# ModelTC/Dipoorlet

Measured on AMD Instinct MI355X. Metric: calibration images/sec (whole node) + achieved HBM GB/s, ResNet-50 ONNX N=1024, -A hist, higher is better.
Workload: dtype f32; 1 GPU; ResNet-50 ONNX activation set (T=123, 26598376 fp32 elems/img), -A hist --bins 2048, N=1024 per GPU in 32 batches of 32: range pass + histogram pass + percentile clip; device=AMD Radeon Graphics (gfx950:sramecc+:xnack-), hist_checksum_ok=True, world_size_seen_by_backend=1

## Files before the change

### dipoorlet_amd/_hip.py

```python
import ctypes as C
import os

import torch

_HERE = os.path.dirname(os.path.abspath(__file__))
LIB_PATH = os.environ.get("DPL_LIB") or os.path.join(_HERE, "csrc", "libdipoorlet_hip.so")

ABI_VERSION = 24
MAX_BINS = 16384
HIST_SPEC_MAX_TENSORS = 2048


class Span(C.Structure):
    _fields_ = [("offset", C.c_uint64), ("count", C.c_uint64), ("seg", C.c_uint32), ("slot", C.c_uint32)]


class WorkItem(C.Structure):
    _fields_ = [("offset", C.c_uint64), ("count", C.c_uint32), ("seg", C.c_uint32), ("slot", C.c_uint32),
                ("reserved", C.c_uint32)]


class HistRange(C.Structure):
    _fields_ = [("first", C.c_float), ("last", C.c_float), ("step", C.c_float), ("inv", C.c_float),
                ("zero_bin", C.c_uint32), ("status", C.c_uint32), ("dmax", C.c_float), ("exact_div", C.c_uint32)]
# ... 44 lines not shown
SIGNATURES = {
    "dpl_abi_version": (C.c_int, []),
    "dpl_last_error": (C.c_char_p, []),
    "dpl_device_info": (C.c_int, [C.c_char_p, C.c_int, C.POINTER(C.c_int), C.POINTER(C.c_uint64)]),
    "dpl_stream_priority_range": (C.c_int, [C.POINTER(C.c_int), C.POINTER(C.c_int)]),
    "dpl_stream_create": (C.c_int, [C.c_int, C.POINTER(C.c_void_p)]),
    "dpl_stream_destroy": (C.c_int, [_P]),
    "dpl_build_work_items": (_I64, [_P, _I64, _U64, _P, _I64]),
    "dpl_build_balanced_items": (_I64, [_P, _I64, _I64, _P, _I64, _P]),
    "dpl_minmax_init": (C.c_int, [_P, _P, _P, _I64, _P]),
    "dpl_minmax_accumulate": (C.c_int, [_P, _I64, _P, _I64, _P, _P, _P, _P, _P]),
    "dpl_minmax_finalize": (C.c_int, [_P, _P, _P, _I64, _P, _P, _P]),
    "dpl_minmax_encode": (C.c_int, [_P, _P, _I64, _P, _P, _P, _P]),
    "dpl_hist_prepare": (C.c_int, [_P, _P, _I64, C.c_int, _P, _P]),
    "dpl_abs_hist_accumulate": (C.c_int, [_P, _I64, _P, _I64, _P, _P, C.c_int, _P, _P]),
    "dpl_hist_spec_entry_bytes": (_U64, [_I64, C.c_int]),
    "dpl_minmax_hist_accumulate": (C.c_int, [_P, _I64, _P, _I64, _P, _P, _P, _P, _I64, C.c_int, _P, _P]),
    "dpl_hist_spec_accumulate": (C.c_int, [_P, _P, _I64, _I64, _P, _P, C.c_int, _P, _P, _P]),
    "dpl_hist_spec_cuts": (C.c_int, [_P, _P, _I64, _I64, _P, _P]),
    "dpl_hist_percentile": (C.c_int, [_P, _P, _P, _I64, C.c_int, _DBL, _P, _P]),
    "dpl_hist_kl": (C.c_int, [_P, _P, _P, _I64, C.c_int, C.c_int, _P, _P, _P, _P]),
    "dpl_octav_init": (C.c_int, [_P, _I64, C.c_int, _P]),
    "dpl_octav_run_compact": (C.c_int, [_P, _I64, _P, _I64, _P, _P, _I64, _P, _P, _P, _P, _P, C.c_int, C.c_int, _P]),
    "dpl_octav_run": (C.c_int, [_P, _I64, _P, _I64, _P, _P, _I64, C.c_int, C.c_int, _P]),
    "dpl_octav_run_bracket": (C.c_int, [_P, _I64, _P, _I64, _P, _P, _I64, _P, _P, _P, _P, _P, _P, _P, _P, C.c_int,
                                        C.c_int, _P]),
    "dpl_octav_slice_cap": (C.c_uint32, []),
    "dpl_octav_small_pair": (C.c_uint32, []),
    "dpl_build_octav_slices": (_I64, [_P, _I64, _P, _I64, _P]),
    "dpl_octav_oneread_prepare": (C.c_int, [_P, _P]),
    "dpl_octav_oneread_stream": (C.c_int, [_P, _P]),
    "dpl_octav_oneread_finish": (C.c_int, [_P, _P]),
    "dpl_octav_oneread_compaction": (C.c_int, [_P, _P]),
# ... 120 lines not shown
```

### dipoorlet_amd/csrc/calib_kernels.hip

```cpp
#include "common.hpp"

#pragma clang fp contract(off)

namespace {

struct MinMaxOp {
    float mn, mx;
    uint32_t nan;
    __device__ __forceinline__ void operator()(float x) {
        mn = fminf(mn, x);
        mx = fmaxf(mx, x);
        nan |= (x != x);
    }
};

__device__ __forceinline__ void minmax_commit(const MinMaxOp& op, uint32_t slot, float* s_mn, float* s_mx, uint32_t* s_nan,
                                              uint32_t* __restrict__ min_enc, uint32_t* __restrict__ max_enc,
                                              uint32_t* __restrict__ nan_flag) {
    float mn = wave_min(op.mn), mx = wave_max(op.mx);
    uint32_t nn = __any(op.nan) ? 1u : 0u;
    const int w = threadIdx.x / kWave;
    if ((threadIdx.x & (kWave - 1)) == 0) {
        s_mn[w] = mn;
        s_mx[w] = mx;
// ... 105 lines not shown
};

template <bool kFast>
__device__ __forceinline__ void hist_op_init(HistOp<kFast>& op, const dpl_hist_range& r, int bins, uint32_t* lds) {
    op.lds = lds;
    op.first = r.first;
    op.last = r.last;
    op.step = r.step;
    op.inv = r.inv;
    op.denom = __fsub_rn(r.last, r.first);
    op.last_bin = bins - 1;
    op.fbins = (float)bins;
    op.nonzero = 0u;
}

template <class Count>
__device__ __forceinline__ void hist_flush(uint32_t nonzero, const dpl_work_item& it, const dpl_hist_range& r, int bins,
                                           Count* __restrict__ hist, uint32_t* lds, uint32_t* s_nz) {
    const uint32_t nzw = wave_sum(nonzero);
    if ((threadIdx.x & (kWave - 1)) == 0) s_nz[threadIdx.x / kWave] = nzw;
    __syncthreads();
    if (threadIdx.x == 0) {
        uint32_t nzb = 0;
        for (int k = 0; k < kBlock / kWave; ++k) nzb += s_nz[k];
        const uint32_t z = it.count - nzb;
        if (z) atomicAdd(lds + r.zero_bin, z);
        const uint32_t top = lds[bins];
        if (top) atomicAdd(lds + bins - 1, top);
    }
    __syncthreads();
    Count* __restrict__ out = hist + (uint64_t)it.slot * (uint64_t)bins;
    for (int b = threadIdx.x; b < bins; b += kBlock) {
        const uint32_t c = lds[b];
        if (c) {
            if constexpr (sizeof(Count) == 8)
                atomicAdd(reinterpret_cast<unsigned long long*>(out + b), (unsigned long long)c);
            else
                atomicAdd(out + b, c);
        }
    }
}

template <bool kFast>
__device__ __forceinline__ void hist_body(const dpl_work_item& it, const float* const* __restrict__ segs,
                                          const dpl_hist_range& r, int bins, uint64_t* __restrict__ hist,
                                          uint32_t* lds, uint32_t* s_nz) {
    HistOp<kFast> op;
    hist_op_init(op, r, bins, lds);
    stream_span(segs[it.seg] + it.offset, it.count, op);
    hist_flush(op.nonzero, it, r, bins, hist, lds, s_nz);
}

__global__ __launch_bounds__(kBlock) void k_abs_hist(const dpl_work_item* __restrict__ items,
                                                      const uint32_t* __restrict__ bb,
                                                      const float* const* __restrict__ segs,
// ... 52 lines not shown
        b = b < 0 ? 0 : b;
        if (a < hist_edge(b, r.step, first)) --b;
        if (b != bins - 1 && a >= hist_edge(b + 1, r.step, first)) ++b;
        r.zero_bin = (uint32_t)(b < 0 ? 0 : b);
    }
    return r;
}

__global__ void k_hist_prepare(const float* __restrict__ gmin, const float* __restrict__ gmax, int64_t n, int bins,
                               dpl_hist_range* __restrict__ out) {
    int64_t i = (int64_t)blockIdx.x * blockDim.x + threadIdx.x;
    if (i >= n) return;
    out[i] = hist_range_of(gmin[i], gmax[i], bins);
}

__host__ __device__ inline uint64_t spec_counts_offset(int64_t n_slots) {
    return (((uint64_t)n_slots * (sizeof(dpl_hist_range) + sizeof(uint32_t))) + 15ull) & ~15ull;
}

__global__ __launch_bounds__(kBlock) void k_hist_snapshot(const uint32_t* __restrict__ mn, const uint32_t* __restrict__ mx,
                                                           const uint32_t* __restrict__ nan, int64_t n, int bins,
                                                           dpl_hist_range* __restrict__ snap, uint32_t* __restrict__ flags,
                                                           uint32_t* __restrict__ counts) {
    const int64_t i = (int64_t)blockIdx.x * blockDim.x + threadIdx.x;
    const int64_t stride = (int64_t)gridDim.x * blockDim.x;
    if (i < n) {
        float gmin, gmax;
        minmax_decode(mn[i], mx[i], nan[i], gmin, gmax);
        snap[i] = hist_range_of(gmin, gmax, bins);
        flags[i] = 0u;
    }
    const int64_t total = n * (int64_t)bins;
    for (int64_t j = i; j < total; j += stride) counts[j] = 0u;
}

template <bool kFast>
struct MinMaxHistOp {
    MinMaxOp m;
    HistOp<kFast> h;
    __device__ __forceinline__ void operator()(float x) {
        m(x);
        h(x);
    }
};

template <bool kFast>
__device__ __forceinline__ void minmax_hist_body(const dpl_work_item& it, const float* const* __restrict__ segs,
                                                 const dpl_hist_range& r, int bins, uint32_t* __restrict__ counts,
                                                 uint32_t* lds, uint32_t* s_nz, MinMaxOp& m) {
    MinMaxHistOp<kFast> op;
    op.m = m;
    hist_op_init(op.h, r, bins, lds);
    stream_span(segs[it.seg] + it.offset, it.count, op);
    m = op.m;
    hist_flush(op.h.nonzero, it, r, bins, counts, lds, s_nz);
}

__global__ __launch_bounds__(kBlock) void k_minmax_hist(const dpl_work_item* __restrict__ items,
                                                         const uint32_t* __restrict__ bb,
                                                         const float* const* __restrict__ segs,
                                                         uint32_t* __restrict__ min_enc, uint32_t* __restrict__ max_enc,
                                                         uint32_t* __restrict__ nan_flag,
                                                         const dpl_hist_range* __restrict__ snap, int bins,
                                                         uint32_t* __restrict__ counts) {
    extern __shared__ __attribute__((aligned(16))) uint32_t lds_mh[];
    uint32_t* s_nz = lds_mh + bins + 1;
    float* s_mn = reinterpret_cast<float*>(s_nz + kBlock / kWave);
    float* s_mx = s_mn + kBlock / kWave;
    uint32_t* s_nan = reinterpret_cast<uint32_t*>(s_mx + kBlock / kWave);
    uint32_t k0, k1;
    block_items(bb, k0, k1);
    for (uint32_t k = k0; k < k1; ++k) {
        const dpl_work_item it = items[k];
        const dpl_hist_range r = snap[it.slot];
        MinMaxOp m{INFINITY, -INFINITY, 0u};
        if (r.status != 0u) {
            stream_span(segs[it.seg] + it.offset, it.count, m);
        } else {
            for (int b = threadIdx.x; b <= bins; b += kBlock) lds_mh[b] = 0u;
            __syncthreads();
            if (r.exact_div)
                minmax_hist_body<false>(it, segs, r, bins, counts, lds_mh, s_nz, m);
            else
                minmax_hist_body<true>(it, segs, r, bins, counts, lds_mh, s_nz, m);
        }
        minmax_commit(m, it.slot, s_mn, s_mx, s_nan, min_enc, max_enc, nan_flag);
    }
}

__global__ __launch_bounds__(kBlock) void k_hist_resolve(const dpl_hist_range* __restrict__ snap,
                                                          const dpl_hist_range* __restrict__ fin,
                                                          const uint32_t* __restrict__ counts, const uint64_t* __restrict__ elems,
                                                          int bins, uint64_t* __restrict__ hist, uint32_t* __restrict__ flags,
                                                          unsigned long long* __restrict__ stats) {
    const uint32_t t = blockIdx.x;
    const uint32_t* a = reinterpret_cast<const uint32_t*>(snap + t);
    const uint32_t* b = reinterpret_cast<const uint32_t*>(fin + t);
    bool same = true;
#pragma unroll
    for (int w = 0; w < (int)(sizeof(dpl_hist_range) / 4); ++w) same = same && (a[w] == b[w]);
    const uint32_t status = fin[t].status;
    const bool valid = same && status == 0u;
    if (threadIdx.x == 0) {
        flags[t] = valid ? 1u : (status != 0u ? 2u : 0u);
        if (stats) {
            const unsigned long long e = elems[t];
            atomicAdd(stats + 0, 1ull);
            atomicAdd(stats + 2, e);
            if (valid) {
                atomicAdd(stats + 1, 1ull);
                atomicAdd(stats + 3, e);
            }
        }
    }
    if (!valid) return;
    const uint32_t* __restrict__ row = counts + (uint64_t)t * (uint64_t)bins;
    uint64_t* __restrict__ out = hist + (uint64_t)t * (uint64_t)bins;
    for (int j = threadIdx.x; j < bins; j += kBlock) {
        const uint32_t c = row[j];
        if (c) out[j] += (uint64_t)c;
    }
}

__device__ __forceinline__ uint64_t shfl_up_u64(uint64_t v, int d) {
    const uint32_t lo = __shfl_up((uint32_t)v, d, kWave), hi = __shfl_up((uint32_t)(v >> 32), d, kWave);
    return ((uint64_t)hi << 32) | lo;
}

__device__ __forceinline__ void rest_prefix(const uint64_t* __restrict__ elems, const uint32_t* __restrict__ flags, int n_tensors,
                                            uint64_t* P, uint64_t* s_tot) {
    const int per = (n_tensors + kBlock - 1) / kBlock;
    const int t0 = (int)threadIdx.x * per;
    uint64_t mine = 0;
    for (int j = 0; j < per; ++j) {
        const int t = t0 + j;
        if (t < n_tensors && flags[t] == 0u) mine += elems[t];
    }
    uint64_t incl = mine;
    const int lane = threadIdx.x & (kWave - 1), wv = threadIdx.x / kWave;
#pragma unroll
    for (int o = 1; o < kWave; o <<= 1) {
        const uint64_t up = shfl_up_u64(incl, o);
        if (lane >= o) incl += up;
    }
    if (lane == kWave - 1) s_tot[wv] = incl;
    __syncthreads();
    uint64_t run = incl - mine;
    for (int w = 0; w < wv; ++w) run += s_tot[w];
    for (int j = 0; j < per; ++j) {
        const int t = t0 + j;
        if (t < n_tensors) {
            P[t] = run;
            if (flags[t] == 0u) run += elems[t];
        }
    }
    if (threadIdx.x == kBlock - 1) P[n_tensors] = run;
    __syncthreads();
}

__device__ __forceinline__ void rest_cut(const uint64_t* P, int n_tensors, uint64_t G, uint64_t b, uint64_t& cut, int& at) {
    const uint64_t total = P[n_tensors], q = total / G, rem = total % G;
    const uint64_t target = (b >= G) ? total : q * b + (rem * b) / G;
    if (target >= total) {
        cut = total;
        at = n_tensors;
        return;
    }
    int lo = 1, hi = n_tensors;
    while (lo < hi) {
        const int mid = (lo + hi) >> 1;
        if (P[mid] > target) hi = mid; else lo = mid + 1;
    }
    at = lo - 1;
    cut = P[lo - 1] + ((target - P[lo - 1]) & ~1023ull);
}

__global__ __launch_bounds__(kBlock) void k_abs_hist_rest(const uint64_t* __restrict__ elems, const uint32_t* __restrict__ flags,
                                                           int n_tensors, const float* const* __restrict__ segs,
                                                           const dpl_hist_range* __restrict__ ranges, int bins,
                                                           uint64_t* __restrict__ hist) {
    extern __shared__ __attribute__((aligned(16))) uint32_t lds_rest[];
    uint64_t* P = reinterpret_cast<uint64_t*>(lds_rest);
    uint64_t* s_tot = P + n_tensors + 1;
    uint32_t* lds = reinterpret_cast<uint32_t*>(s_tot + kBlock / kWave);
    uint32_t* s_nz = lds + bins + 1;
    rest_prefix(elems, flags, n_tensors, P, s_tot);
    if (P[n_tensors] == 0) return;
    uint64_t cut[2];
    int at[2];
    rest_cut(P, n_tensors, gridDim.x, blockIdx.x, cut[0], at[0]);
    rest_cut(P, n_tensors, gridDim.x, (uint64_t)blockIdx.x + 1, cut[1], at[1]);
    uint64_t pos = cut[0];
    const uint64_t end = cut[1];
    int t = at[0];
    while (pos < end) {
        while (P[t + 1] <= pos) ++t;
        const uint64_t stop = P[t + 1] < end ? P[t + 1] : end;
        dpl_work_item it;
        it.offset = pos - P[t];
        it.count = (uint32_t)(stop - pos);
        it.seg = (uint32_t)t;
// ... 4 lines not shown
        __syncthreads();
        if (r.exact_div)
            hist_body<false>(it, segs, r, bins, hist, lds, s_nz);
        else
            hist_body<true>(it, segs, r, bins, hist, lds, s_nz);
        __syncthreads();
        pos = stop;
    }
}

__global__ __launch_bounds__(kBlock) void k_hist_spec_cuts(const uint64_t* __restrict__ elems, const uint32_t* __restrict__ flags,
                                                            int n_tensors, uint64_t* __restrict__ cuts) {
    extern __shared__ __attribute__((aligned(16))) uint32_t lds_cuts[];
    uint64_t* P = reinterpret_cast<uint64_t*>(lds_cuts);
    uint64_t* s_tot = P + n_tensors + 1;
    rest_prefix(elems, flags, n_tensors, P, s_tot);
    if (threadIdx.x != 0) return;
    uint64_t cut = 0;
    int at = 0;
    if (P[n_tensors] != 0) rest_cut(P, n_tensors, gridDim.x, blockIdx.x, cut, at);
    cuts[blockIdx.x] = cut;
    if (blockIdx.x + 1 == gridDim.x) cuts[gridDim.x] = P[n_tensors];
}

__device__ __forceinline__ void store_bin_clip(int found, float gmin, float gmax, int bins, float* __restrict__ clip) {
    float lo = gmin, hi = gmax;
    if (found >= 0) {
        const float dmax = py_max(-gmin, gmax);
        const float cv = __fmul_rn((float)found + 0.5f, __fdiv_rn(dmax, (float)bins));
        lo = py_max(-cv, gmin);
        hi = py_min(cv, gmax);
// ... 767 lines not shown
}

int dpl_abs_hist_accumulate(const dpl_work_item* d_items, int64_t n_items, const uint32_t* d_block_begin,
                            int64_t n_blocks, const float* const* d_seg_ptrs, const dpl_hist_range* d_ranges,
                            int bins, uint64_t* d_hist, dpl_stream_t s) {
    if (bins < 1 || bins > DPL_MAX_BINS) return fail_msg("dpl_abs_hist_accumulate: bins must be in [1, 16384]");
    if (n_items <= 0) return 0;
    if (int e = check_blocks("dpl_abs_hist_accumulate", n_items, d_block_begin, n_blocks)) return e;
    hipLaunchKernelGGL(k_abs_hist, dim3((unsigned)n_blocks), dim3(kBlock),
                       ((size_t)bins + 1 + kBlock / kWave) * sizeof(uint32_t), (hipStream_t)s, d_items, d_block_begin,
                       d_seg_ptrs, d_ranges, bins, d_hist);
    DPL_LAUNCH_CHECK("k_abs_hist");
    return 0;
}

uint64_t dpl_hist_spec_entry_bytes(int64_t n_slots, int bins) {
    if (n_slots < 0 || bins < 1 || bins > DPL_MAX_BINS) return 0;
    return spec_counts_offset(n_slots) + (uint64_t)n_slots * (uint64_t)bins * sizeof(uint32_t);
}

int dpl_minmax_hist_accumulate(const dpl_work_item* d_items, int64_t n_items, const uint32_t* d_block_begin,
                               int64_t n_blocks, const float* const* d_seg_ptrs, uint32_t* d_min_enc, uint32_t* d_max_enc,
                               uint32_t* d_nan, int64_t n_slots, int bins, void* d_entry, dpl_stream_t s) {
    if (bins < 1 || bins > DPL_MAX_BINS) return fail_msg("dpl_minmax_hist_accumulate: bins must be in [1, 16384]");
    if (!d_entry || ((uintptr_t)d_entry & 15u)) return fail_msg("dpl_minmax_hist_accumulate: d_entry must be 16-byte aligned");
    if (n_slots <= 0 || n_slots > 0x7FFFFFFFll) return fail_msg("dpl_minmax_hist_accumulate: n_slots out of range");
    if (n_items <= 0) return 0;
    if (int e = check_blocks("dpl_minmax_hist_accumulate", n_items, d_block_begin, n_blocks)) return e;
    dpl_hist_range* snap = (dpl_hist_range*)d_entry;
    uint32_t* flags = (uint32_t*)(snap + n_slots);
    uint32_t* counts = (uint32_t*)((char*)d_entry + spec_counts_offset(n_slots));
    int64_t zb = grid_for(n_slots * (int64_t)bins, kBlock * 8);
    if (zb < grid_for(n_slots, kBlock)) zb = grid_for(n_slots, kBlock);
    if (zb > 1024) zb = 1024;
    hipLaunchKernelGGL(k_hist_snapshot, dim3((unsigned)zb), dim3(kBlock), 0, (hipStream_t)s, d_min_enc, d_max_enc, d_nan,
                       n_slots, bins, snap, flags, counts);
    DPL_LAUNCH_CHECK("k_hist_snapshot");
    hipLaunchKernelGGL(k_minmax_hist, dim3((unsigned)n_blocks), dim3(kBlock),
                       ((size_t)bins + 1 + 4 * (kBlock / kWave)) * sizeof(uint32_t), (hipStream_t)s, d_items, d_block_begin,
                       d_seg_ptrs, d_min_enc, d_max_enc, d_nan, snap, bins, counts);
    DPL_LAUNCH_CHECK("k_minmax_hist");
    return 0;
}

int dpl_hist_spec_accumulate(void* d_entry, const uint64_t* d_elems, int64_t n_slots, int64_t n_blocks,
                             const float* const* d_seg_ptrs, const dpl_hist_range* d_ranges, int bins, uint64_t* d_hist,
                             uint64_t* d_stats, dpl_stream_t s) {
    if (bins < 1 || bins > DPL_MAX_BINS) return fail_msg("dpl_hist_spec_accumulate: bins must be in [1, 16384]");
    if (!d_entry || ((uintptr_t)d_entry & 15u)) return fail_msg("dpl_hist_spec_accumulate: d_entry must be 16-byte aligned");
    if (n_slots <= 0 || n_slots > DPL_HIST_SPEC_MAX_TENSORS)
        return fail_msg("dpl_hist_spec_accumulate: n_slots must be in [1, DPL_HIST_SPEC_MAX_TENSORS]");
    if (n_blocks <= 0 || n_blocks > 0x7FFFFFFFll) return fail_msg("dpl_hist_spec_accumulate: n_blocks out of range");
    dpl_hist_range* snap = (dpl_hist_range*)d_entry;
    uint32_t* flags = (uint32_t*)(snap + n_slots);
    const uint32_t* counts = (const uint32_t*)((char*)d_entry + spec_counts_offset(n_slots));
    hipLaunchKernelGGL(k_hist_resolve, dim3((unsigned)n_slots), dim3(kBlock), 0, (hipStream_t)s, snap, d_ranges, counts, d_elems,
                       bins, d_hist, flags, (unsigned long long*)d_stats);
    DPL_LAUNCH_CHECK("k_hist_resolve");
    const size_t lds = ((size_t)n_slots + 1 + kBlock / kWave) * sizeof(uint64_t) + ((size_t)bins + 1 + kBlock / kWave) * sizeof(uint32_t);
    hipLaunchKernelGGL(k_abs_hist_rest, dim3((unsigned)n_blocks), dim3(kBlock), lds, (hipStream_t)s, d_elems, flags, (int)n_slots,
                       d_seg_ptrs, d_ranges, bins, d_hist);
    DPL_LAUNCH_CHECK("k_abs_hist_rest");
    return 0;
}

int dpl_hist_spec_cuts(const void* d_entry, const uint64_t* d_elems, int64_t n_slots, int64_t n_blocks, uint64_t* d_cuts,
                       dpl_stream_t s) {
    if (!d_entry || !d_cuts) return fail_msg("dpl_hist_spec_cuts: null argument");
    if (n_slots <= 0 || n_slots > DPL_HIST_SPEC_MAX_TENSORS)
        return fail_msg("dpl_hist_spec_cuts: n_slots must be in [1, DPL_HIST_SPEC_MAX_TENSORS]");
    if (n_blocks <= 0 || n_blocks > 0x7FFFFFFFll) return fail_msg("dpl_hist_spec_cuts: n_blocks out of range");
    const uint32_t* flags = (const uint32_t*)((const dpl_hist_range*)d_entry + n_slots);
    hipLaunchKernelGGL(k_hist_spec_cuts, dim3((unsigned)n_blocks), dim3(kBlock),
                       ((size_t)n_slots + 1 + kBlock / kWave) * sizeof(uint64_t), (hipStream_t)s, d_elems, flags, (int)n_slots, d_cuts);
    DPL_LAUNCH_CHECK("k_hist_spec_cuts");
    return 0;
// ... 117 lines not shown
```

### dipoorlet_amd/ops.py

```python
import ctypes as C
import os
import weakref

import numpy as np
import torch

from . import _hip

_SEG_CACHE_MAX = 64


def _stream():
    return C.c_void_p(torch.cuda.current_stream().cuda_stream)


def _ptr(t):
    return C.c_void_p(t.data_ptr())


def _require_cuda(t, name="tensor"):
    if not (isinstance(t, torch.Tensor) and t.is_cuda):
        raise _hip.DipoorletHipError(f"{name} must be a ROCm device tensor; dipoorlet_amd has no CPU path")
    if t.dtype != torch.float32 or not t.is_contiguous():
        raise _hip.DipoorletHipError(f"{name} must be contiguous float32")


def _upload_struct_array(arr, n, device):
    nbytes = C.sizeof(arr._type_) * max(n, 1)
    host = torch.frombuffer(bytearray(C.string_at(C.addressof(arr), nbytes)), dtype=torch.uint8)
    return host.to(device)


DEFAULT_BLOCKS = {"minmax": 256, "hist": 768, "octav": 1024, "cos": 512, "fq": 65536}


class WorkSet:

    def __init__(self, items, n_items, block_begin, n_blocks):
        self.items, self.n_items, self.block_begin, self.n_blocks = items, n_items, block_begin, n_blocks

    def args(self):
        bb = _ptr(self.block_begin) if self.block_begin is not None else C.c_void_p(0)
        return _ptr(self.items), self.n_items, bb, self.n_blocks


class TensorSetPlan:

    def __init__(self, elems_per_image, batch, device, chunk_elems=None):
# ... 3 lines not shown
        self.device = torch.device(device)
        self.total = sum(self.elems) * self.batch
        self.chunk = int(chunk_elems) if chunk_elems else None
        self._work = {}
        self._seg_cache = {}

    @property
    def n_pairs(self):
        return self.batch * self.T

    def _spans(self, per_image):
        if per_image:
            return [(t, b * e, e, b * self.T + t) for b in range(self.batch) for t, e in enumerate(self.elems)]
        return [(t, 0, e * self.batch, t) for t, e in enumerate(self.elems)]

    def work(self, kind, per_image=False):
        nb = None if self.chunk else max(1, min(DEFAULT_BLOCKS[kind], (self.total + 4095) // 4096))
        key = (per_image, nb)
        w = self._work.get(key)
        if w is None:
            spans = self._spans(per_image)
            if self.chunk:
                arr, n = _hip.build_work_items(spans, self.chunk)
                w = WorkSet(_upload_struct_array(arr, n, self.device), n, None, n)
            else:
                arr, n, bb = _hip.build_balanced_items(spans, nb)
                bbt = torch.frombuffer(bytearray(bytes(bb)), dtype=torch.int32).to(self.device)
                w = WorkSet(_upload_struct_array(arr, n, self.device), n, bbt, nb)
            self._work[key] = w
        return w

    def elems_device(self):
# ... 195 lines not shown
            raise _hip.DipoorletHipError(f"bins must be in [1, {_hip.MAX_BINS}]")
        self.min_enc = torch.empty(self.n, dtype=torch.int32, device=self.device)
        self.max_enc = torch.empty(self.n, dtype=torch.int32, device=self.device)
        self.nan = torch.empty(self.n, dtype=torch.int32, device=self.device)
        self.gmin = torch.empty(self.n, dtype=torch.float32, device=self.device)
        self.gmax = torch.empty(self.n, dtype=torch.float32, device=self.device)
        self.hist = None
        self.ranges = None
        self.speculate = bool(speculate)
        self._ledger = {}
        self._slab = []
        self._spec_stats = torch.zeros(4, dtype=torch.int64, device=self.device) if self.speculate else None
        self.reset_minmax()

    def reset_minmax(self):
        for _, entry, _ in self._ledger.values():
            self._slab.append(entry)
        self._ledger.clear()
        _hip.check(_hip.lib().dpl_minmax_init(_ptr(self.min_enc), _ptr(self.max_enc), _ptr(self.nan), self.n,
                                              _stream()), "dpl_minmax_init")

    def will_speculate(self, plan, tensors, per_image=False):
        return (self.speculate and isinstance(tensors, BoundSet) and not per_image and plan.chunk is None
                and 0 < plan.T <= min(self.n, _hip.HIST_SPEC_MAX_TENSORS)
                and max(plan.elems) * plan.batch < (1 << 32)
                and plan.T * self.bins * 4 * self.SPEC_MAX_SHARE <= plan.total * 4)

    def _entry_for(self, bound):
        rec = self._ledger.get(id(bound))
        if rec is not None and rec[0]() is bound:
            return rec[1]
        if self._slab:
            entry = self._slab.pop()
        else:
            nbytes = int(_hip.lib().dpl_hist_spec_entry_bytes(self.n, self.bins))
            entry = torch.empty(nbytes, dtype=torch.uint8, device=self.device)
        key, slab, ledger = id(bound), self._slab, self._ledger

        def dropped(ref):
            rec = ledger.get(key)
            if rec is not None and rec[0] is ref:
                del ledger[key]
                slab.append(rec[1])
        self._ledger[key] = (weakref.ref(bound, dropped), entry, bound.plan.T)
        return entry

    def _entry_of(self, plan, tensors):
        if not isinstance(tensors, BoundSet):
            return None
        rec = self._ledger.get(id(tensors))
        if rec is None or rec[0]() is not tensors or rec[2] != plan.T:
            return None
        return rec[1]

    def spec_stats(self, reset=False):
        v = [0, 0, 0, 0] if self._spec_stats is None else [int(x) for x in self._spec_stats.cpu().tolist()]
        if reset and self._spec_stats is not None:
            self._spec_stats.zero_()
        return dict(zip(("pairs", "pairs_skipped", "elements", "elements_skipped"), v))

    def spec_flags(self, tensors):
        rec = self._ledger.get(id(tensors))
        if rec is None or rec[0]() is not tensors:
            return None
        T = rec[2]
        off = T * C.sizeof(_hip.HistRange)
        return rec[1][off:off + 4 * T].view(torch.int32).cpu()

    def spec_cuts(self, plan, tensors):
        entry = self._entry_of(plan, tensors)
        if entry is None:
            return None
        nb = plan.work("hist").n_blocks
        out = torch.empty(nb + 1, dtype=torch.int64, device=self.device)
        _hip.check(_hip.lib().dpl_hist_spec_cuts(_ptr(entry), _ptr(plan.elems_device()), plan.T, nb, _ptr(out), _stream()),
                   "dpl_hist_spec_cuts")
        return out.cpu()

    def minmax_accumulate(self, plan, tensors, per_image=False):
        tab = plan.seg_table(tensors)
        if self.n < (plan.n_pairs if per_image else plan.T):
            raise _hip.DipoorletHipError("accumulator has fewer slots than the plan addresses")
        if self.will_speculate(plan, tensors, per_image):
            w = plan.work("hist")
            entry = self._entry_for(tensors)
            plan.elems_device()
            _hip.check(_hip.lib().dpl_minmax_hist_accumulate(*w.args(), _ptr(tab), _ptr(self.min_enc), _ptr(self.max_enc),
                                                             _ptr(self.nan), plan.T, self.bins, _ptr(entry), _stream()),
                       "dpl_minmax_hist_accumulate")
            return
        if isinstance(tensors, BoundSet):
            rec = self._ledger.get(id(tensors))
            if rec is not None and rec[0]() is tensors:
                del self._ledger[id(tensors)]
                self._slab.append(rec[1])
        w = plan.work("minmax", per_image)
        _hip.check(_hip.lib().dpl_minmax_accumulate(*w.args(), _ptr(tab), _ptr(self.min_enc), _ptr(self.max_enc),
                                                    _ptr(self.nan), _stream()), "dpl_minmax_accumulate")

    def finalize_minmax(self):
# ... 8 lines not shown
        _hip.check(_hip.lib().dpl_minmax_encode(_ptr(self.gmin), _ptr(self.gmax), self.n, _ptr(self.min_enc),
                                                _ptr(self.max_enc), _ptr(self.nan), _stream()), "dpl_minmax_encode")

    def hist_prepare(self):
        if self.hist is None:
            self.hist = torch.zeros(self.n, self.bins, dtype=torch.int64, device=self.device)
            self.ranges = torch.empty(self.n * C.sizeof(_hip.HistRange), dtype=torch.uint8, device=self.device)
        else:
            self.hist.zero_()
        _hip.check(_hip.lib().dpl_hist_prepare(_ptr(self.gmin), _ptr(self.gmax), self.n, self.bins,
                                               _ptr(self.ranges), _stream()), "dpl_hist_prepare")

    def abs_hist_accumulate(self, plan, tensors):
        tab = plan.seg_table(tensors)
        w = plan.work("hist")
        entry = self._entry_of(plan, tensors)
        if entry is not None:
            _hip.check(_hip.lib().dpl_hist_spec_accumulate(_ptr(entry), _ptr(plan.elems_device()), plan.T, w.n_blocks, _ptr(tab),
                                                           _ptr(self.ranges), self.bins, _ptr(self.hist), _ptr(self._spec_stats),
                                                           _stream()), "dpl_hist_spec_accumulate")
            return
        _hip.check(_hip.lib().dpl_abs_hist_accumulate(*w.args(), _ptr(tab), _ptr(self.ranges), self.bins,
                                                      _ptr(self.hist), _stream()), "dpl_abs_hist_accumulate")

    def range_status(self):
        raw = self.ranges.cpu().numpy().view(np.dtype([("first", "<f4"), ("last", "<f4"), ("step", "<f4"),
                                                       ("inv", "<f4"), ("zero_bin", "<u4"), ("status", "<u4"),
                                                       ("dmax", "<f4"), ("exact_div", "<u4")]))
        return raw

    def hist_percentile(self, threshold):
        clip = torch.empty(self.n, 2, dtype=torch.float32, device=self.device)
        _hip.check(_hip.lib().dpl_hist_percentile(_ptr(self.hist), _ptr(self.gmin), _ptr(self.gmax), self.n,
                                                  self.bins, float(threshold), _ptr(clip), _stream()),
                   "dpl_hist_percentile")
# ... 494 lines not shown
```

### include/dipoorlet_hip.h

```cpp
#ifndef DIPOORLET_HIP_H
#define DIPOORLET_HIP_H

#include <stdint.h>

#ifdef __cplusplus
extern "C" {
#endif

#define DPL_ABI_VERSION 24
#define DPL_MAX_BINS 16384
#define DPL_HIST_SPEC_MAX_TENSORS 2048

typedef void* dpl_stream_t;

typedef struct dpl_span {
    uint64_t offset;
    uint64_t count;
    uint32_t seg;
    uint32_t slot;
} dpl_span;

typedef struct dpl_work_item {
    uint64_t offset;
    uint32_t count;
// ... 41 lines not shown

int dpl_minmax_init(uint32_t* d_min_enc, uint32_t* d_max_enc, uint32_t* d_nan, int64_t n_slots, dpl_stream_t s);
int dpl_minmax_accumulate(const dpl_work_item* d_items, int64_t n_items, const uint32_t* d_block_begin,
                          int64_t n_blocks, const float* const* d_seg_ptrs, uint32_t* d_min_enc,
                          uint32_t* d_max_enc, uint32_t* d_nan, dpl_stream_t s);
int dpl_minmax_finalize(const uint32_t* d_min_enc, const uint32_t* d_max_enc, const uint32_t* d_nan,
                        int64_t n_slots, float* d_min, float* d_max, dpl_stream_t s);
int dpl_minmax_encode(const float* d_min, const float* d_max, int64_t n_slots, uint32_t* d_min_enc,
                      uint32_t* d_max_enc, uint32_t* d_nan, dpl_stream_t s);

int dpl_hist_prepare(const float* d_min, const float* d_max, int64_t n_slots, int bins,
                     dpl_hist_range* d_ranges, dpl_stream_t s);
int dpl_abs_hist_accumulate(const dpl_work_item* d_items, int64_t n_items, const uint32_t* d_block_begin,
                            int64_t n_blocks, const float* const* d_seg_ptrs, const dpl_hist_range* d_ranges,
                            int bins, uint64_t* d_hist, dpl_stream_t s);
uint64_t dpl_hist_spec_entry_bytes(int64_t n_slots, int bins);
int dpl_minmax_hist_accumulate(const dpl_work_item* d_items, int64_t n_items, const uint32_t* d_block_begin,
                               int64_t n_blocks, const float* const* d_seg_ptrs, uint32_t* d_min_enc, uint32_t* d_max_enc,
                               uint32_t* d_nan, int64_t n_slots, int bins, void* d_entry, dpl_stream_t s);
int dpl_hist_spec_accumulate(void* d_entry, const uint64_t* d_elems, int64_t n_slots, int64_t n_blocks,
                             const float* const* d_seg_ptrs, const dpl_hist_range* d_ranges, int bins, uint64_t* d_hist,
                             uint64_t* d_stats, dpl_stream_t s);
int dpl_hist_spec_cuts(const void* d_entry, const uint64_t* d_elems, int64_t n_slots, int64_t n_blocks, uint64_t* d_cuts,
                       dpl_stream_t s);
int dpl_hist_percentile(const uint64_t* d_hist, const float* d_min, const float* d_max, int64_t n_slots,
                        int bins, double threshold, float* d_clip, dpl_stream_t s);

int dpl_hist_kl(const uint64_t* d_hist, const float* d_min, const float* d_max, int64_t n_slots, int bins,
                int levels, double* d_div, int32_t* d_best, float* d_clip, dpl_stream_t s);

int dpl_octav_init(dpl_octav_state* d_states, int64_t n_pairs, int list_mode, dpl_stream_t s);
int dpl_octav_run(const dpl_work_item* d_items, int64_t n_items, const uint32_t* d_block_begin, int64_t n_blocks,
                  const float* const* d_seg_ptrs, dpl_octav_state* d_states, int64_t n_pairs, int dynamic_sym,
                  int max_iters, dpl_stream_t s);
int dpl_octav_run_compact(const dpl_work_item* d_items, int64_t n_items, const uint32_t* d_block_begin,
                          int64_t n_blocks, const float* const* d_seg_ptrs, dpl_octav_state* d_states,
// ... 159 lines not shown
```

Before: 58180 images/s.

## Write per-item private histogram rows instead of global atomics in speculative minmax-hist

The fused minmax+histogram pass now writes each work item's LDS histogram to a private row, so the snapshot kernel no longer zeroes a shared counts buffer and the pass issues no global atomics. The resolve step moves into the rest kernel, which reduces each tensor's rows in LDS before adding them to the final histogram. A separate minmax_hist block count caps the number of rows relative to the bin count, which bounds scratch size. The cost is more scratch memory and an extra reduction read of the rows, plus a linear scan of the item list for each tensor.

```diff
diff --git a/dipoorlet_amd/_hip.py b/dipoorlet_amd/_hip.py
--- a/dipoorlet_amd/_hip.py
+++ b/dipoorlet_amd/_hip.py
@@ -6,7 +6,7 @@
 _HERE = os.path.dirname(os.path.abspath(__file__))
 LIB_PATH = os.environ.get("DPL_LIB") or os.path.join(_HERE, "csrc", "libdipoorlet_hip.so")
 
-ABI_VERSION = 24
+ABI_VERSION = 25
 MAX_BINS = 16384
 HIST_SPEC_MAX_TENSORS = 2048
 
@@ -82,9 +82,9 @@
     "dpl_minmax_encode": (C.c_int, [_P, _P, _I64, _P, _P, _P, _P]),
     "dpl_hist_prepare": (C.c_int, [_P, _P, _I64, C.c_int, _P, _P]),
     "dpl_abs_hist_accumulate": (C.c_int, [_P, _I64, _P, _I64, _P, _P, C.c_int, _P, _P]),
-    "dpl_hist_spec_entry_bytes": (_U64, [_I64, C.c_int]),
+    "dpl_hist_spec_entry_bytes": (_U64, [_I64, _I64, C.c_int]),
     "dpl_minmax_hist_accumulate": (C.c_int, [_P, _I64, _P, _I64, _P, _P, _P, _P, _I64, C.c_int, _P, _P]),
-    "dpl_hist_spec_accumulate": (C.c_int, [_P, _P, _I64, _I64, _P, _P, C.c_int, _P, _P, _P]),
+    "dpl_hist_spec_accumulate": (C.c_int, [_P, _P, _I64, _P, _I64, _I64, _P, _P, C.c_int, _P, _P, _P]),
     "dpl_hist_spec_cuts": (C.c_int, [_P, _P, _I64, _I64, _P, _P]),
     "dpl_hist_percentile": (C.c_int, [_P, _P, _P, _I64, C.c_int, _DBL, _P, _P]),
     "dpl_hist_kl": (C.c_int, [_P, _P, _P, _I64, C.c_int, C.c_int, _P, _P, _P, _P]),
diff --git a/dipoorlet_amd/csrc/calib_kernels.hip b/dipoorlet_amd/csrc/calib_kernels.hip
--- a/dipoorlet_amd/csrc/calib_kernels.hip
+++ b/dipoorlet_amd/csrc/calib_kernels.hip
@@ -143,9 +143,8 @@
     op.nonzero = 0u;
 }
 
-template <class Count>
-__device__ __forceinline__ void hist_flush(uint32_t nonzero, const dpl_work_item& it, const dpl_hist_range& r, int bins,
-                                           Count* __restrict__ hist, uint32_t* lds, uint32_t* s_nz) {
+__device__ __forceinline__ void hist_fold(uint32_t nonzero, const dpl_work_item& it, const dpl_hist_range& r, int bins,
+                                          uint32_t* lds, uint32_t* s_nz) {
     const uint32_t nzw = wave_sum(nonzero);
     if ((threadIdx.x & (kWave - 1)) == 0) s_nz[threadIdx.x / kWave] = nzw;
     __syncthreads();
@@ -158,16 +157,22 @@
         if (top) atomicAdd(lds + bins - 1, top);
     }
     __syncthreads();
-    Count* __restrict__ out = hist + (uint64_t)it.slot * (uint64_t)bins;
+}
+
+__device__ __forceinline__ void hist_flush(uint32_t nonzero, const dpl_work_item& it, const dpl_hist_range& r, int bins,
+                                           uint64_t* __restrict__ hist, uint32_t* lds, uint32_t* s_nz) {
+    hist_fold(nonzero, it, r, bins, lds, s_nz);
+    uint64_t* __restrict__ out = hist + (uint64_t)it.slot * (uint64_t)bins;
     for (int b = threadIdx.x; b < bins; b += kBlock) {
         const uint32_t c = lds[b];
-        if (c) {
-            if constexpr (sizeof(Count) == 8)
-                atomicAdd(reinterpret_cast<unsigned long long*>(out + b), (unsigned long long)c);
-            else
-                atomicAdd(out + b, c);
-        }
-    }
+        if (c) atomicAdd(reinterpret_cast<unsigned long long*>(out + b), (unsigned long long)c);
+    }
+}
+
+__device__ __forceinline__ void hist_store_row(uint32_t nonzero, const dpl_work_item& it, const dpl_hist_range& r, int bins,
+                                               uint32_t* __restrict__ row, uint32_t* lds, uint32_t* s_nz) {
+    hist_fold(nonzero, it, r, bins, lds, s_nz);
+    for (int b = threadIdx.x; b < bins; b += kBlock) row[b] = lds[b];
 }
 
 template <bool kFast>
@@ -250,24 +255,20 @@
     out[i] = hist_range_of(gmin[i], gmax[i], bins);
 }
 
-__host__ __device__ inline uint64_t spec_counts_offset(int64_t n_slots) {
+__host__ __device__ inline uint64_t spec_rows_offset(int64_t n_slots) {
     return (((uint64_t)n_slots * (sizeof(dpl_hist_range) + sizeof(uint32_t))) + 15ull) & ~15ull;
 }
 
 __global__ __launch_bounds__(kBlock) void k_hist_snapshot(const uint32_t* __restrict__ mn, const uint32_t* __restrict__ mx,
                                                            const uint32_t* __restrict__ nan, int64_t n, int bins,
-                                                           dpl_hist_range* __restrict__ snap, uint32_t* __restrict__ flags,
-                                                           uint32_t* __restrict__ counts) {
+                                                           dpl_hist_range* __restrict__ snap, uint32_t* __restrict__ flags) {
     const int64_t i = (int64_t)blockIdx.x * blockDim.x + threadIdx.x;
-    const int64_t stride = (int64_t)gridDim.x * blockDim.x;
     if (i < n) {
         float gmin, gmax;
         minmax_decode(mn[i], mx[i], nan[i], gmin, gmax);
         snap[i] = hist_range_of(gmin, gmax, bins);
         flags[i] = 0u;
     }
-    const int64_t total = n * (int64_t)bins;
-    for (int64_t j = i; j < total; j += stride) counts[j] = 0u;
 }
 
 template <bool kFast>
@@ -282,14 +283,14 @@
 
 template <bool kFast>
 __device__ __forceinline__ void minmax_hist_body(const dpl_work_item& it, const float* const* __restrict__ segs,
-                                                 const dpl_hist_range& r, int bins, uint32_t* __restrict__ counts,
+                                                 const dpl_hist_range& r, int bins, uint32_t* __restrict__ row,
                                                  uint32_t* lds, uint32_t* s_nz, MinMaxOp& m) {
     MinMaxHistOp<kFast> op;
     op.m = m;
     hist_op_init(op.h, r, bins, lds);
     stream_span(segs[it.seg] + it.offset, it.count, op);
     m = op.m;
-    hist_flush(op.h.nonzero, it, r, bins, counts, lds, s_nz);
+    hist_store_row(op.h.nonzero, it, r, bins, row, lds, s_nz);
 }
 
 __global__ __launch_bounds__(kBlock) void k_minmax_hist(const dpl_work_item* __restrict__ items,
@@ -298,7 +299,7 @@
                                                          uint32_t* __restrict__ min_enc, uint32_t* __restrict__ max_enc,
                                                          uint32_t* __restrict__ nan_flag,
                                                          const dpl_hist_range* __restrict__ snap, int bins,
-                                                         uint32_t* __restrict__ counts) {
+                                                         uint32_t* __restrict__ rows) {
     extern __shared__ __attribute__((aligned(16))) uint32_t lds_mh[];
     uint32_t* s_nz = lds_mh + bins + 1;
     float* s_mn = reinterpret_cast<float*>(s_nz + kBlock / kWave);
@@ -315,62 +316,53 @@
         } else {
             for (int b = threadIdx.x; b <= bins; b += kBlock) lds_mh[b] = 0u;
             __syncthreads();
+            uint32_t* __restrict__ row = rows + (uint64_t)k * (uint64_t)bins;
             if (r.exact_div)
-                minmax_hist_body<false>(it, segs, r, bins, counts, lds_mh, s_nz, m);
+                minmax_hist_body<false>(it, segs, r, bins, row, lds_mh, s_nz, m);
             else
-                minmax_hist_body<true>(it, segs, r, bins, counts, lds_mh, s_nz, m);
+                minmax_hist_body<true>(it, segs, r, bins, row, lds_mh, s_nz, m);
         }
         minmax_commit(m, it.slot, s_mn, s_mx, s_nan, min_enc, max_enc, nan_flag);
     }
 }
 
-__global__ __launch_bounds__(kBlock) void k_hist_resolve(const dpl_hist_range* __restrict__ snap,
-                                                          const dpl_hist_range* __restrict__ fin,
-                                                          const uint32_t* __restrict__ counts, const uint64_t* __restrict__ elems,
-                                                          int bins, uint64_t* __restrict__ hist, uint32_t* __restrict__ flags,
-                                                          unsigned long long* __restrict__ stats) {
-    const uint32_t t = blockIdx.x;
-    const uint32_t* a = reinterpret_cast<const uint32_t*>(snap + t);
-    const uint32_t* b = reinterpret_cast<const uint32_t*>(fin + t);
+__device__ __forceinline__ bool range_same(const dpl_hist_range* __restrict__ a, const dpl_hist_range* __restrict__ b) {
+    const uint32_t* x = reinterpret_cast<const uint32_t*>(a);
+    const uint32_t* y = reinterpret_cast<const uint32_t*>(b);
     bool same = true;
 #pragma unroll
-    for (int w = 0; w < (int)(sizeof(dpl_hist_range) / 4); ++w) same = same && (a[w] == b[w]);
-    const uint32_t status = fin[t].status;
-    const bool valid = same && status == 0u;
-    if (threadIdx.x == 0) {
-        flags[t] = valid ? 1u : (status != 0u ? 2u : 0u);
-        if (stats) {
-            const unsigned long long e = elems[t];
-            atomicAdd(stats + 0, 1ull);
-            atomicAdd(stats + 2, e);
-            if (valid) {
-                atomicAdd(stats + 1, 1ull);
-                atomicAdd(stats + 3, e);
-            }
-        }
-    }
-    if (!valid) return;
-    const uint32_t* __restrict__ row = counts + (uint64_t)t * (uint64_t)bins;
-    uint64_t* __restrict__ out = hist + (uint64_t)t * (uint64_t)bins;
-    for (int j = threadIdx.x; j < bins; j += kBlock) {
-        const uint32_t c = row[j];
-        if (c) out[j] += (uint64_t)c;
-    }
-}
+    for (int w = 0; w < (int)(sizeof(dpl_hist_range) / 4); ++w) same = same && (x[w] == y[w]);
+    return same;
+}
+
+struct RestByFlags {
+    const uint32_t* __restrict__ flags;
+    __device__ __forceinline__ bool operator()(int t) const { return flags[t] == 0u; }
+};
+struct RestByRange {
+    const dpl_hist_range* __restrict__ snap;
+    const dpl_hist_range* __restrict__ fin;
+    __device__ __forceinline__ bool operator()(int t) const { return fin[t].status == 0u && !range_same(snap + t, fin + t); }
+};
 
 __device__ __forceinline__ uint64_t shfl_up_u64(uint64_t v, int d) {
     const uint32_t lo = __shfl_up((uint32_t)v, d, kWave), hi = __shfl_up((uint32_t)(v >> 32), d, kWave);
     return ((uint64_t)hi << 32) | lo;
 }
 
-__device__ __forceinline__ void rest_prefix(const uint64_t* __restrict__ elems, const uint32_t* __restrict__ flags, int n_tensors,
+template <class Rest>
+__device__ __forceinline__ void rest_prefix(const uint64_t* __restrict__ elems, const Rest rest, int n_tensors,
                                             uint64_t* P, uint64_t* s_tot) {
     const int per = (n_tensors + kBlock - 1) / kBlock;
     const int t0 = (int)threadIdx.x * per;
     uint64_t mine = 0;
     for (int j = 0; j < per; ++j) {
         const int t = t0 + j;
-        if (t < n_tensors && flags[t] == 0u) mine += elems[t];
+        if (t < n_tensors) {
+            const uint64_t e = rest(t) ? elems[t] : 0ull;
+            P[t] = e;
+            mine += e;
+        }
     }
     uint64_t incl = mine;
     const int lane = threadIdx.x & (kWave - 1), wv = threadIdx.x / kWave;
@@ -386,8 +378,9 @@
     for (int j = 0; j < per; ++j) {
         const int t = t0 + j;
         if (t < n_tensors) {
+            const uint64_t e = P[t];
             P[t] = run;
-            if (flags[t] == 0u) run += elems[t];
+            run += e;
         }
     }
     if (threadIdx.x == kBlock - 1) P[n_tensors] = run;
@@ -411,16 +404,82 @@
     cut = P[lo - 1] + ((target - P[lo - 1]) & ~1023ull);
 }
 
-__global__ __launch_bounds__(kBlock) void k_abs_hist_rest(const uint64_t* __restrict__ elems, const uint32_t* __restrict__ flags,
+__global__ __launch_bounds__(kBlock) void k_abs_hist_rest(const uint64_t* __restrict__ elems, const dpl_hist_range* __restrict__ snap,
+                                                           uint32_t* __restrict__ flags, const uint32_t* __restrict__ rows,
+                                                           const dpl_work_item* __restrict__ r_items, uint32_t n_r_items,
                                                            int n_tensors, const float* const* __restrict__ segs,
                                                            const dpl_hist_range* __restrict__ ranges, int bins,
-                                                           uint64_t* __restrict__ hist) {
+                                                           uint64_t* __restrict__ hist, unsigned long long* __restrict__ stats) {
     extern __shared__ __attribute__((aligned(16))) uint32_t lds_rest[];
     uint64_t* P = reinterpret_cast<uint64_t*>(lds_rest);
     uint64_t* s_tot = P + n_tensors + 1;
     uint32_t* lds = reinterpret_cast<uint32_t*>(s_tot + kBlock / kWave);
     uint32_t* s_nz = lds + bins + 1;
-    rest_prefix(elems, flags, n_tensors, P, s_tot);
+    __shared__ uint32_t s_row[2];
+    for (uint32_t t = blockIdx.x; t < (uint32_t)n_tensors; t += gridDim.x) {
+        const uint32_t status = ranges[t].status;
+        const bool valid = status == 0u && range_same(snap + t, ranges + t);
+        if (threadIdx.x == 0) {
+            flags[t] = valid ? 1u : (status != 0u ? 2u : 0u);
+            if (stats) {
+                const unsigned long long e = elems[t];
+                atomicAdd(stats + 0, 1ull);
+                atomicAdd(stats + 2, e);
+                if (valid) {
+                    atomicAdd(stats + 1, 1ull);
+                    atomicAdd(stats + 3, e);
+                }
+            }
+            s_row[0] = s_row[1] = 0u;
+        }
+        if (!valid) continue;
+        __syncthreads();
+        for (uint32_t k = threadIdx.x; k < n_r_items; k += kBlock) {
+            if (r_items[k].slot != t) continue;
+            if (k == 0 || r_items[k - 1].slot != t) s_row[0] = k;
+            if (k + 1 == n_r_items || r_items[k + 1].slot != t) s_row[1] = k + 1;
+        }
+        __syncthreads();
+        const uint32_t first = s_row[0], end = s_row[1];
+        for (int b = threadIdx.x; b < bins; b += kBlock) lds[b] = 0u;
+        __syncthreads();
+        const uint32_t* __restrict__ base = rows + (uint64_t)first * (uint64_t)bins;
+        const uint64_t n = (uint64_t)(end - first) * (uint64_t)bins;
+        if ((bins & 3) == 0) {
+            const uint4* __restrict__ v = reinterpret_cast<const uint4*>(base);
+            const uint32_t q = (uint32_t)bins >> 2, step = kBlock % q;
+            uint32_t col = threadIdx.x % q;
+#pragma unroll 8
+            for (uint64_t i = threadIdx.x; i < (n >> 2); i += kBlock) {
+                const uint4 c = v[i];
+                uint32_t* dst = lds + 4u * col;
+                if (c.x) atomicAdd(dst + 0, c.x);
+                if (c.y) atomicAdd(dst + 1, c.y);
+                if (c.z) atomicAdd(dst + 2, c.z);
+                if (c.w) atomicAdd(dst + 3, c.w);
+                col += step;
+                col -= col >= q ? q : 0u;
+            }
+        } else {
+            const uint32_t q = (uint32_t)bins, step = kBlock % q;
+            uint32_t col = threadIdx.x % q;
+#pragma unroll 8
+            for (uint64_t i = threadIdx.x; i < n; i += kBlock) {
+                const uint32_t c = base[i];
+                if (c) atomicAdd(lds + col, c);
+                col += step;
+                col -= col >= q ? q : 0u;
+            }
+        }
+        __syncthreads();
+        uint64_t* __restrict__ out = hist + (uint64_t)t * (uint64_t)bins;
+        for (int b = threadIdx.x; b < bins; b += kBlock) {
+            const uint32_t c = lds[b];
+            if (c) out[b] += (uint64_t)c;
+        }
+        __syncthreads();
+    }
+    rest_prefix(elems, RestByRange{snap, ranges}, n_tensors, P, s_tot);
     if (P[n_tensors] == 0) return;
     uint64_t cut[2];
     int at[2];
@@ -455,7 +514,7 @@
     extern __shared__ __attribute__((aligned(16))) uint32_t lds_cuts[];
     uint64_t* P = reinterpret_cast<uint64_t*>(lds_cuts);
     uint64_t* s_tot = P + n_tensors + 1;
-    rest_prefix(elems, flags, n_tensors, P, s_tot);
+    rest_prefix(elems, RestByFlags{flags}, n_tensors, P, s_tot);
     if (threadIdx.x != 0) return;
     uint64_t cut = 0;
     int at = 0;
@@ -1253,9 +1312,9 @@
     return 0;
 }
 
-uint64_t dpl_hist_spec_entry_bytes(int64_t n_slots, int bins) {
-    if (n_slots < 0 || bins < 1 || bins > DPL_MAX_BINS) return 0;
-    return spec_counts_offset(n_slots) + (uint64_t)n_slots * (uint64_t)bins * sizeof(uint32_t);
+uint64_t dpl_hist_spec_entry_bytes(int64_t n_slots, int64_t n_items, int bins) {
+    if (n_slots < 0 || n_items < 0 || bins < 1 || bins > DPL_MAX_BINS) return 0;
+    return spec_rows_offset(n_slots) + (uint64_t)n_items * (uint64_t)bins * sizeof(uint32_t);
 }
 
 int dpl_minmax_hist_accumulate(const dpl_work_item* d_items, int64_t n_items, const uint32_t* d_block_begin,
@@ -1265,40 +1324,38 @@
     if (!d_entry || ((uintptr_t)d_entry & 15u)) return fail_msg("dpl_minmax_hist_accumulate: d_entry must be 16-byte aligned");
     if (n_slots <= 0 || n_slots > 0x7FFFFFFFll) return fail_msg("dpl_minmax_hist_accumulate: n_slots out of range");
     if (n_items <= 0) return 0;
+    if (n_items > 0x7FFFFFFFll) return fail_msg("dpl_minmax_hist_accumulate: n_items out of range");
     if (int e = check_blocks("dpl_minmax_hist_accumulate", n_items, d_block_begin, n_blocks)) return e;
     dpl_hist_range* snap = (dpl_hist_range*)d_entry;
     uint32_t* flags = (uint32_t*)(snap + n_slots);
-    uint32_t* counts = (uint32_t*)((char*)d_entry + spec_counts_offset(n_slots));
-    int64_t zb = grid_for(n_slots * (int64_t)bins, kBlock * 8);
-    if (zb < grid_for(n_slots, kBlock)) zb = grid_for(n_slots, kBlock);
-    if (zb > 1024) zb = 1024;
-    hipLaunchKernelGGL(k_hist_snapshot, dim3((unsigned)zb), dim3(kBlock), 0, (hipStream_t)s, d_min_enc, d_max_enc, d_nan,
-                       n_slots, bins, snap, flags, counts);
+    uint32_t* rows = (uint32_t*)((char*)d_entry + spec_rows_offset(n_slots));
+    hipLaunchKernelGGL(k_hist_snapshot, dim3(grid_for(n_slots, kBlock)), dim3(kBlock), 0, (hipStream_t)s, d_min_enc, d_max_enc, d_nan,
+                       n_slots, bins, snap, flags);
     DPL_LAUNCH_CHECK("k_hist_snapshot");
     hipLaunchKernelGGL(k_minmax_hist, dim3((unsigned)n_blocks), dim3(kBlock),
                        ((size_t)bins + 1 + 4 * (kBlock / kWave)) * sizeof(uint32_t), (hipStream_t)s, d_items, d_block_begin,
-                       d_seg_ptrs, d_min_enc, d_max_enc, d_nan, snap, bins, counts);
+                       d_seg_ptrs, d_min_enc, d_max_enc, d_nan, snap, bins, rows);
     DPL_LAUNCH_CHECK("k_minmax_hist");
     return 0;
 }
 
-int dpl_hist_spec_accumulate(void* d_entry, const uint64_t* d_elems, int64_t n_slots, int64_t n_blocks,
-                             const float* const* d_seg_ptrs, const dpl_hist_range* d_ranges, int bins, uint64_t* d_hist,
+int dpl_hist_spec_accumulate(void* d_entry, const dpl_work_item* d_range_items, int64_t n_range_items, const uint64_t* d_elems,
+                             int64_t n_slots, int64_t n_blocks, const float* const* d_seg_ptrs, const dpl_hist_range* d_ranges, int bins, uint64_t* d_hist,
                              uint64_t* d_stats, dpl_stream_t s) {
     if (bins < 1 || bins > DPL_MAX_BINS) return fail_msg("dpl_hist_spec_accumulate: bins must be in [1, 16384]");
     if (!d_entry || ((uintptr_t)d_entry & 15u)) return fail_msg("dpl_hist_spec_accumulate: d_entry must be 16-byte aligned");
     if (n_slots <= 0 || n_slots > DPL_HIST_SPEC_MAX_TENSORS)
         return fail_msg("dpl_hist_spec_accumulate: n_slots must be in [1, DPL_HIST_SPEC_MAX_TENSORS]");
     if (n_blocks <= 0 || n_blocks > 0x7FFFFFFFll) return fail_msg("dpl_hist_spec_accumulate: n_blocks out of range");
+    if (n_range_items < 0 || n_range_items > 0x7FFFFFFFll || (n_range_items > 0 && !d_range_items))
+        return fail_msg("dpl_hist_spec_accumulate: the range pass's items are missing or out of range");
     dpl_hist_range* snap = (dpl_hist_range*)d_entry;
     uint32_t* flags = (uint32_t*)(snap + n_slots);
-    const uint32_t* counts = (const uint32_t*)((char*)d_entry + spec_counts_offset(n_slots));
-    hipLaunchKernelGGL(k_hist_resolve, dim3((unsigned)n_slots), dim3(kBlock), 0, (hipStream_t)s, snap, d_ranges, counts, d_elems,
-                       bins, d_hist, flags, (unsigned long long*)d_stats);
-    DPL_LAUNCH_CHECK("k_hist_resolve");
+    const uint32_t* rows = (const uint32_t*)((char*)d_entry + spec_rows_offset(n_slots));
     const size_t lds = ((size_t)n_slots + 1 + kBlock / kWave) * sizeof(uint64_t) + ((size_t)bins + 1 + kBlock / kWave) * sizeof(uint32_t);
-    hipLaunchKernelGGL(k_abs_hist_rest, dim3((unsigned)n_blocks), dim3(kBlock), lds, (hipStream_t)s, d_elems, flags, (int)n_slots,
-                       d_seg_ptrs, d_ranges, bins, d_hist);
+    hipLaunchKernelGGL(k_abs_hist_rest, dim3((unsigned)n_blocks), dim3(kBlock), lds, (hipStream_t)s, d_elems, snap, flags, rows,
+                       d_range_items, (uint32_t)n_range_items, (int)n_slots, d_seg_ptrs, d_ranges, bins, d_hist,
+                       (unsigned long long*)d_stats);
     DPL_LAUNCH_CHECK("k_abs_hist_rest");
     return 0;
 }
diff --git a/dipoorlet_amd/ops.py b/dipoorlet_amd/ops.py
--- a/dipoorlet_amd/ops.py
+++ b/dipoorlet_amd/ops.py
@@ -31,7 +31,7 @@
     return host.to(device)
 
 
-DEFAULT_BLOCKS = {"minmax": 256, "hist": 768, "octav": 1024, "cos": 512, "fq": 65536}
+DEFAULT_BLOCKS = {"minmax": 256, "hist": 768, "minmax_hist": 768, "octav": 1024, "cos": 512, "fq": 65536}
 
 
 class WorkSet:
@@ -65,8 +65,10 @@
             return [(t, b * e, e, b * self.T + t) for b in range(self.batch) for t, e in enumerate(self.elems)]
         return [(t, 0, e * self.batch, t) for t, e in enumerate(self.elems)]
 
-    def work(self, kind, per_image=False):
+    def work(self, kind, per_image=False, bins=None):
         nb = None if self.chunk else max(1, min(DEFAULT_BLOCKS[kind], (self.total + 4095) // 4096))
+        if kind == "minmax_hist" and nb is not None:
+            nb = max(1, min(nb, (self.total * 4) // (64 * int(bins) * 4)))
         key = (per_image, nb)
         w = self._work.get(key)
         if w is None:
@@ -292,8 +294,8 @@
         self.reset_minmax()
 
     def reset_minmax(self):
-        for _, entry, _ in self._ledger.values():
-            self._slab.append(entry)
+        for rec in self._ledger.values():
+            self._slab.append(rec[1])
         self._ledger.clear()
         _hip.check(_hip.lib().dpl_minmax_init(_ptr(self.min_enc), _ptr(self.max_enc), _ptr(self.nan), self.n,
                                               _stream()), "dpl_minmax_init")
@@ -304,14 +306,20 @@
                 and max(plan.elems) * plan.batch < (1 << 32)
                 and plan.T * self.bins * 4 * self.SPEC_MAX_SHARE <= plan.total * 4)
 
-    def _entry_for(self, bound):
+    def _entry_for(self, bound, w):
+        T = bound.plan.T
+        nbytes = int(_hip.lib().dpl_hist_spec_entry_bytes(T, w.n_items, self.bins))
         rec = self._ledger.get(id(bound))
         if rec is not None and rec[0]() is bound:
-            return rec[1]
-        if self._slab:
-            entry = self._slab.pop()
+            if rec[1].numel() >= nbytes:
+                self._ledger[id(bound)] = (rec[0], rec[1], T, w)
+                return rec[1]
+            del self._ledger[id(bound)]
+            self._slab.append(rec[1])
+        fit = next((i for i in range(len(self._slab) - 1, -1, -1) if self._slab[i].numel() >= nbytes), None)
+        if fit is not None:
+            entry = self._slab.pop(fit)
         else:
-            nbytes = int(_hip.lib().dpl_hist_spec_entry_bytes(self.n, self.bins))
             entry = torch.empty(nbytes, dtype=torch.uint8, device=self.device)
         key, slab, ledger = id(bound), self._slab, self._ledger
 
@@ -320,7 +328,7 @@
             if rec is not None and rec[0] is ref:
                 del ledger[key]
                 slab.append(rec[1])
-        self._ledger[key] = (weakref.ref(bound, dropped), entry, bound.plan.T)
+        self._ledger[key] = (weakref.ref(bound, dropped), entry, T, w)
         return entry
 
     def _entry_of(self, plan, tensors):
@@ -329,7 +337,7 @@
         rec = self._ledger.get(id(tensors))
         if rec is None or rec[0]() is not tensors or rec[2] != plan.T:
             return None
-        return rec[1]
+        return rec[1], rec[3]
 
     def spec_stats(self, reset=False):
         v = [0, 0, 0, 0] if self._spec_stats is None else [int(x) for x in self._spec_stats.cpu().tolist()]
@@ -346,9 +354,10 @@
         return rec[1][off:off + 4 * T].view(torch.int32).cpu()
 
     def spec_cuts(self, plan, tensors):
-        entry = self._entry_of(plan, tensors)
-        if entry is None:
+        found = self._entry_of(plan, tensors)
+        if found is None:
             return None
+        entry = found[0]
         nb = plan.work("hist").n_blocks
         out = torch.empty(nb + 1, dtype=torch.int64, device=self.device)
         _hip.check(_hip.lib().dpl_hist_spec_cuts(_ptr(entry), _ptr(plan.elems_device()), plan.T, nb, _ptr(out), _stream()),
@@ -360,8 +369,8 @@
         if self.n < (plan.n_pairs if per_image else plan.T):
             raise _hip.DipoorletHipError("accumulator has fewer slots than the plan addresses")
         if self.will_speculate(plan, tensors, per_image):
-            w = plan.work("hist")
-            entry = self._entry_for(tensors)
+            w = plan.work("minmax_hist", bins=self.bins)
+            entry = self._entry_for(tensors, w)
             plan.elems_device()
             _hip.check(_hip.lib().dpl_minmax_hist_accumulate(*w.args(), _ptr(tab), _ptr(self.min_enc), _ptr(self.max_enc),
                                                              _ptr(self.nan), plan.T, self.bins, _ptr(entry), _stream()),
@@ -400,11 +409,12 @@
     def abs_hist_accumulate(self, plan, tensors):
         tab = plan.seg_table(tensors)
         w = plan.work("hist")
-        entry = self._entry_of(plan, tensors)
-        if entry is not None:
-            _hip.check(_hip.lib().dpl_hist_spec_accumulate(_ptr(entry), _ptr(plan.elems_device()), plan.T, w.n_blocks, _ptr(tab),
-                                                           _ptr(self.ranges), self.bins, _ptr(self.hist), _ptr(self._spec_stats),
-                                                           _stream()), "dpl_hist_spec_accumulate")
+        found = self._entry_of(plan, tensors)
+        if found is not None:
+            entry, rw = found
+            _hip.check(_hip.lib().dpl_hist_spec_accumulate(_ptr(entry), _ptr(rw.items), rw.n_items, _ptr(plan.elems_device()), plan.T,
+                                                           w.n_blocks, _ptr(tab), _ptr(self.ranges), self.bins, _ptr(self.hist),
+                                                           _ptr(self._spec_stats), _stream()), "dpl_hist_spec_accumulate")
             return
         _hip.check(_hip.lib().dpl_abs_hist_accumulate(*w.args(), _ptr(tab), _ptr(self.ranges), self.bins,
                                                       _ptr(self.hist), _stream()), "dpl_abs_hist_accumulate")
diff --git a/include/dipoorlet_hip.h b/include/dipoorlet_hip.h
--- a/include/dipoorlet_hip.h
+++ b/include/dipoorlet_hip.h
@@ -7,7 +7,7 @@
 extern "C" {
 #endif
 
-#define DPL_ABI_VERSION 24
+#define DPL_ABI_VERSION 25
 #define DPL_MAX_BINS 16384
 #define DPL_HIST_SPEC_MAX_TENSORS 2048
 
@@ -79,12 +79,12 @@
 int dpl_abs_hist_accumulate(const dpl_work_item* d_items, int64_t n_items, const uint32_t* d_block_begin,
                             int64_t n_blocks, const float* const* d_seg_ptrs, const dpl_hist_range* d_ranges,
                             int bins, uint64_t* d_hist, dpl_stream_t s);
-uint64_t dpl_hist_spec_entry_bytes(int64_t n_slots, int bins);
+uint64_t dpl_hist_spec_entry_bytes(int64_t n_slots, int64_t n_items, int bins);
 int dpl_minmax_hist_accumulate(const dpl_work_item* d_items, int64_t n_items, const uint32_t* d_block_begin,
                                int64_t n_blocks, const float* const* d_seg_ptrs, uint32_t* d_min_enc, uint32_t* d_max_enc,
                                uint32_t* d_nan, int64_t n_slots, int bins, void* d_entry, dpl_stream_t s);
-int dpl_hist_spec_accumulate(void* d_entry, const uint64_t* d_elems, int64_t n_slots, int64_t n_blocks,
-                             const float* const* d_seg_ptrs, const dpl_hist_range* d_ranges, int bins, uint64_t* d_hist,
+int dpl_hist_spec_accumulate(void* d_entry, const dpl_work_item* d_range_items, int64_t n_range_items, const uint64_t* d_elems,
+                             int64_t n_slots, int64_t n_blocks, const float* const* d_seg_ptrs, const dpl_hist_range* d_ranges, int bins, uint64_t* d_hist,
                              uint64_t* d_stats, dpl_stream_t s);
 int dpl_hist_spec_cuts(const void* d_entry, const uint64_t* d_elems, int64_t n_slots, int64_t n_blocks, uint64_t* d_cuts,
                        dpl_stream_t s);
```

Measured after the change: 56860 images/s. 0.977x the previous value.
